# pytorch/torchdistx

Hardware: AMD Instinct MI355X
Metric: deferred_init_materialize_params_per_s (higher is better)
Workload: dtype bf16; 1 GPU; model=llama3-70b, n_params=70553706496, mode=replicate, init=fast, threads=1, replay=pertensor, device=cuda, native_init_kernels=True, parallelism=replicate1

## Files before the change

### torchdistx_amd/csrc/core/deferred_init.cc

```cpp

#include "deferred_init.h"

#include <algorithm>
#include <atomic>
#include <cmath>
#include <condition_variable>
#include <cstring>
#include <functional>
#include <limits>
#include <memory>
#include <mutex>
#include <optional>
#include <unordered_set>
#include <vector>

#include <ATen/CPUGeneratorImpl.h>
#include <ATen/Context.h>
#include <ATen/ThreadLocalState.h>
#include <c10/core/GradMode.h>
#include <ATen/core/dispatch/Dispatcher.h>
#include <ATen/core/VariableHooksInterface.h>
#include <c10/core/DefaultDtype.h>
#include <c10/core/impl/LocalDispatchKeySet.h>
#include <torch/library.h>

#include "box_geometry.h"
#include "fake.h"
#include "native_redirect.h"
#include "stack_utils.h"

namespace tdx {
namespace {

constexpr c10::DispatchKey kDeferredKey = c10::DispatchKey::DeferredInit;
constexpr c10::DispatchKey kFakeKey = c10::DispatchKey::Fake;

struct OpNode;

struct OpOutputDescriptor {
  std::shared_ptr<OpNode> node;
  size_t index = 0;
};

struct AliasGroup {
  std::vector<std::shared_ptr<OpNode>> writers;
};

struct TensorRecord {
  OpOutputDescriptor desc;
  std::shared_ptr<AliasGroup> group;
};

struct RecordedOp {
  std::string name;
  std::function<void(torch::jit::Stack&)> run;
  std::vector<c10::IValue> args;
  at::ThreadLocalState tls;
  std::optional<std::pair<uint64_t, uint64_t>> philox;
  std::optional<c10::OperatorHandle> handle;
};

constexpr uint64_t kPhiloxStridePerOp = 4;

struct RngSession {
  bool has_segment = false;
  uint64_t segment_hash = 0;
  uint64_t nonce = 0;
  uint64_t next_slot = 1;
  std::vector<uint64_t> raw_hashes;
  at::Tensor replay_cursor;
  std::mutex cursor_mutex;
};

thread_local std::shared_ptr<RngSession> current_rng_session;

std::mutex segment_registry_mutex;
std::unordered_map<uint64_t, uint64_t> live_segment_uses;

uint64_t mixSalt(uint64_t h, uint64_t salt) {
  for (int b = 0; b < 8; ++b) {
    h = (h ^ ((salt >> (8 * b)) & 0xff)) * 1099511628211ull;
  }
  return h;
}

bool isRngOpName(const std::string& name) {
  return name == "aten::uniform_" || name == "aten::normal_" ||
         name == "aten::bernoulli_";
}

uint64_t hashStateBytes(const uint8_t* bytes, int64_t n) {
  uint64_t h = 0x9E3779B97F4A7C15ull ^ static_cast<uint64_t>(n);
  int64_t i = 0;
  for (; i + 8 <= n; i += 8) {
    uint64_t w;
    std::memcpy(&w, bytes + i, 8);
    h ^= w;
    h *= 0xBF58476D1CE4E5B9ull;
    h ^= h >> 29;
  }
  uint64_t tail = 0;
  for (int j = 0; i < n; ++i, ++j) {
    tail |= static_cast<uint64_t>(bytes[i]) << (8 * j);
  }
  h ^= tail;
  h *= 0x94D049BB133111EBull;
  h ^= h >> 32;
  return h;
}

void beginRngSession() {
  current_rng_session = std::make_shared<RngSession>();
}

void endRngSession() {
  std::lock_guard<std::mutex> reg_lock(segment_registry_mutex);
  if (current_rng_session != nullptr) {
    for (uint64_t h : current_rng_session->raw_hashes) {
      auto it = live_segment_uses.find(h);
      if (it != live_segment_uses.end() && --(it->second) == 0) {
        live_segment_uses.erase(it);
      }
    }
  }
  current_rng_session = nullptr;
  auto gen = at::globalContext().defaultGenerator(c10::DeviceType::CPU);
  std::lock_guard<std::mutex> lock(gen.mutex());
  gen.get<at::CPUGeneratorImpl>()->random64();
}

std::optional<std::pair<uint64_t, uint64_t>> pinPhiloxForOp(
    const std::string& name, at::Tensor* segment_start) {
  if (!isRngOpName(name) || current_rng_session == nullptr) {
    return std::nullopt;
  }
  RngSession& session = *current_rng_session;
  std::lock_guard<std::mutex> reg_lock(segment_registry_mutex);
  auto gen = at::globalContext().defaultGenerator(c10::DeviceType::CPU);
  at::Tensor state;
  {
    std::lock_guard<std::mutex> lock(gen.mutex());
    state = gen.get_state();
  }
  const uint64_t h =
      hashStateBytes(state.const_data_ptr<uint8_t>(), state.numel());
  if (!session.has_segment || h != session.segment_hash) {
    session.has_segment = true;
    session.segment_hash = h;
    session.next_slot = 1;
    const uint64_t salt = live_segment_uses[h]++;
    session.raw_hashes.push_back(h);
    session.nonce = salt == 0 ? h : mixSalt(h, salt);
    if (salt != 0) {
      auto salted = at::make_generator<at::CPUGeneratorImpl>(session.nonce);
      state = salted.get_state();
    }
    *segment_start = std::move(state);
  }
  return std::make_pair(session.nonce,
                        session.next_slot++ * kPhiloxStridePerOp);
}

struct InputSlot {
  std::optional<OpOutputDescriptor> desc;
  std::optional<uint32_t> external_version;
  std::vector<std::shared_ptr<OpNode>> history;
  bool inference = false;
};

struct AliasGroup;

struct OpNode {
  uint64_t op_nr = 0;
  std::optional<RecordedOp> op;
  std::vector<InputSlot> input_slots;
  std::vector<c10::Storage> output_storages;
  struct OutputMeta {
    c10::ScalarType dtype = c10::ScalarType::Undefined;
    c10::Device device{c10::DeviceType::CPU};
    bool contiguous = false;
    int64_t storage_offset = 0;
    int64_t numel = 0;
  };
  std::vector<OutputMeta> output_metas;
  std::weak_ptr<OpNode> set_data_prior;
  std::vector<std::weak_ptr<OpNode>> dependents;
  std::vector<std::weak_ptr<AliasGroup>> write_groups;
  std::vector<at::Tensor> outputs;
  bool materialized = false;
  bool running = false;
};

std::atomic<uint64_t> next_op_nr{1};

std::recursive_mutex tape_mutex;
std::condition_variable_any tape_cv;

std::shared_ptr<TensorRecord> getRecord(FakeTensorImpl* fake) {
  return std::static_pointer_cast<TensorRecord>(fake->getData(kDeferredKey));
}

void setRecord(FakeTensorImpl* fake, std::shared_ptr<TensorRecord> rec) {
  fake->setData(kDeferredKey, std::move(rec));
}

uint32_t tensorVersion(const at::Tensor& t) {
  return t.unsafeGetTensorImpl()->version_counter().current_version();
}

bool storagesAlias(const c10::Storage& a, const c10::Storage& b) {
  return a && b && a.is_alias_of(b);
}


thread_local size_t deferred_level = 0;

bool shouldRecordHere() {
  return deferred_level > 0 &&
         !c10::impl::tls_is_dispatch_key_excluded(kDeferredKey);
}

void recordOp(std::string name,
              std::function<void(torch::jit::Stack&)> run,
              std::vector<c10::IValue> args,
              at::ThreadLocalState tls,
              torch::jit::Stack& stack,
              size_t rets_begin,
              std::optional<std::pair<uint64_t, uint64_t>> philox =
                  std::nullopt,
              std::optional<c10::OperatorHandle> handle = std::nullopt,
              std::weak_ptr<OpNode> set_data_prior = {}) {
  std::lock_guard<std::recursive_mutex> lock{tape_mutex};
  auto node = std::make_shared<OpNode>();
  node->set_data_prior = std::move(set_data_prior);
  node->op_nr = next_op_nr.fetch_add(1, std::memory_order_relaxed);

  std::vector<std::shared_ptr<TensorRecord>> input_records;
  std::vector<c10::Storage> input_storages;
  std::vector<size_t> fake_slot_idx;
  {
    torch::jit::Stack args_stack{args.begin(), args.end()};
    mapTensors(args_stack, 0, args_stack.size(),
               [&](const at::Tensor& t) -> at::Tensor {
                 if (auto* fake = asFake(t)) {
                   auto rec = getRecord(fake);
                   TORCH_CHECK(
                       rec != nullptr,
                       "A fake tensor constructed outside of a deferred-init "
                       "context (or stripped of its record) was used in `",
                       name, "` and cannot be recorded.");
                   fake_slot_idx.push_back(node->input_slots.size());
                   node->input_slots.push_back(InputSlot{rec->desc, {}, {}});
                   rec->desc.node->dependents.emplace_back(node);
                   input_records.push_back(std::move(rec));
                   input_storages.push_back(fake->meta_tensor().storage());
                   return at::Tensor{};
                 }
                 if (t.defined() && t.is_inference()) {
                   InputSlot slot;
                   slot.inference = true;
                   node->input_slots.push_back(std::move(slot));
                 } else if (t.defined()) {
                   node->input_slots.push_back(
                       InputSlot{{}, tensorVersion(t), {}});
                 } else {
                   node->input_slots.push_back(InputSlot{});
                 }
                 return t;
               });
    args.assign(args_stack.begin(), args_stack.end());
  }

  node->op = RecordedOp{std::move(name), std::move(run), std::move(args),
                        std::move(tls), philox, std::move(handle)};

  visitTensors(stack, rets_begin, stack.size(), [&](const at::Tensor& t) {
    size_t out_idx = node->output_storages.size();
    auto* fake = asFake(t);
    if (fake == nullptr) {
      node->output_storages.emplace_back();
      node->output_metas.emplace_back();
      return;
    }
    const c10::Storage& out_storage = fake->meta_tensor().storage();
    node->output_storages.push_back(out_storage);
    node->output_metas.push_back(OpNode::OutputMeta{
        fake->meta_tensor().scalar_type(), fake->fake_device(),
        fake->meta_tensor().is_contiguous(),
        fake->meta_tensor().storage_offset(), fake->meta_tensor().numel()});

    auto rec = getRecord(fake);
    if (rec == nullptr) {
      rec = std::make_shared<TensorRecord>();
      setRecord(fake, rec);
    }
    rec->desc = OpOutputDescriptor{node, out_idx};

    if (rec->group == nullptr) {
      for (size_t i = 0; i < input_records.size(); ++i) {
        if (storagesAlias(out_storage, input_storages[i]) &&
            input_records[i]->group != nullptr) {
          rec->group = input_records[i]->group;
          break;
        }
      }
      if (rec->group == nullptr) {
        rec->group = std::make_shared<AliasGroup>();
      }
    }
    if (rec->group->writers.empty() ||
        rec->group->writers.back() != node) {
      rec->group->writers.push_back(node);
      node->write_groups.emplace_back(rec->group);
    }
  });

  for (size_t i = 0; i < input_records.size(); ++i) {
    bool writes_it = false;
    for (const c10::Storage& out : node->output_storages) {
      if (storagesAlias(out, input_storages[i])) {
        writes_it = true;
        break;
      }
// ... 337 lines not shown
  recordOp(
      "tdx::set_data",
      [](torch::jit::Stack& s) {
        at::Tensor nd = s.back().toTensor();
        s.pop_back();
        at::Tensor slf = s.back().toTensor();
        s.pop_back();
        slf.set_data(nd);
        s.emplace_back(slf);
      },
      std::move(args), at::ThreadLocalState{}, rets, 0, std::nullopt,
      std::nullopt, std::move(prior));
}


bool outputsAlias(const OpNode& node, const c10::Storage& storage) {
  for (const c10::Storage& s : node.output_storages) {
    if (storagesAlias(s, storage)) {
      return true;
    }
  }
  return false;
}

struct CallStack {
  std::vector<std::shared_ptr<OpNode>> nodes;
  std::unordered_set<OpNode*> members;

  void addWithDeps(const std::shared_ptr<OpNode>& n) {
    if (!members.insert(n.get()).second) {
      return;
    }
    nodes.push_back(n);
    for (const InputSlot& slot : n->input_slots) {
      if (slot.desc.has_value()) {
        addWithDeps(slot.desc->node);
      }
      for (const auto& h : slot.history) {
        addWithDeps(h);
      }
    }
    for (const auto& wg : n->write_groups) {
      if (auto group = wg.lock()) {
        for (const auto& w : group->writers) {
          if (w->op_nr < n->op_nr) {
            addWithDeps(w);
          }
        }
      }
    }
  }
};

std::vector<std::shared_ptr<OpNode>> buildCallStack(const TensorRecord& rec) {
  CallStack cs;
  uint64_t horizon = 0;
  if (rec.group != nullptr) {
    for (const auto& w : rec.group->writers) {
      horizon = std::max(horizon, w->op_nr);
      cs.addWithDeps(w);
    }
  } else {
    cs.addWithDeps(rec.desc.node);
    horizon = rec.desc.node->op_nr;
  }

  bool changed = true;
  while (changed) {
    changed = false;
    std::vector<std::shared_ptr<OpNode>> snapshot = cs.nodes;
    for (const auto& n : snapshot) {
      for (const auto& wd : n->dependents) {
        auto d = wd.lock();
        if (!d || cs.members.count(d.get()) != 0 || d->materialized ||
            d->op_nr > horizon) {
          continue;
        }
        bool include = false;
        for (const InputSlot& slot : d->input_slots) {
          if (!slot.desc.has_value() ||
              cs.members.count(slot.desc->node.get()) == 0) {
            continue;
          }
          const c10::Storage& s =
              slot.desc->node->output_storages[slot.desc->index];
          if (!s) {
            continue;
          }
          for (const auto& w : cs.nodes) {
            if (w->op_nr > d->op_nr && w.get() != slot.desc->node.get() &&
                outputsAlias(*w, s)) {
              include = true;
              break;
            }
          }
          if (include) {
            break;
          }
        }
        if (include) {
          cs.addWithDeps(d);
          changed = true;
        }
      }
    }
  }

  std::sort(cs.nodes.begin(), cs.nodes.end(),
            [](const auto& a, const auto& b) { return a->op_nr < b->op_nr; });
  return cs.nodes;
}

torch::jit::Stack materializeArguments(OpNode& node) {
  torch::jit::Stack stack{node.op->args.begin(), node.op->args.end()};
  size_t visit = 0;
  mapTensors(stack, 0, stack.size(), [&](const at::Tensor& t) -> at::Tensor {
    const InputSlot& slot = node.input_slots.at(visit++);
    if (slot.desc.has_value()) {
      const OpOutputDescriptor& dep = *slot.desc;
      TORCH_INTERNAL_ASSERT(dep.node->materialized,
                            "deferred-init replay ordering bug: dependency "
                            "not yet materialized");
      return dep.node->outputs.at(dep.index);
    }
    TORCH_CHECK(!slot.inference,
                "An inference tensor was used while recording `",
                node.op->name,
                "`; in-place updates to inference tensors cannot be "
                "tracked, so the tape cannot be replayed faithfully.");
    if (t.defined() && slot.external_version.has_value()) {
      TORCH_CHECK(tensorVersion(t) == *slot.external_version,
                  "The external tensor used by the recorded op `",
                  node.op->name,
                  "` was modified in place after recording; the tape can no "
                  "longer be replayed faithfully.");
    }
    return t;
  });
  return stack;
}

void replayNode(std::unique_lock<std::recursive_mutex>& lock,
                const std::shared_ptr<OpNode>& node) {
  while (node->running) {
    tape_cv.wait(lock);
  }
  if (node->materialized) {
    return;
  }
  TORCH_CHECK(node->op.has_value(),
              "This deferred-init tape segment has already been freed and "
              "cannot be replayed again.");
  torch::jit::Stack stack = materializeArguments(*node);
  node->running = true;
  lock.unlock();
  try {
    at::ThreadLocalStateGuard tls_guard{node->op->tls};
    c10::impl::ExcludeDispatchKeyGuard no_deferred{kDeferredKey};
    c10::impl::ExcludeDispatchKeyGuard no_fake{kFakeKey};
    node->op->run(stack);
  } catch (...) {
    lock.lock();
    node->running = false;
    tape_cv.notify_all();
    throw;
  }
  lock.lock();
  node->running = false;
  node->outputs.clear();
  visitTensors(stack, 0, stack.size(),
               [&](const at::Tensor& t) { node->outputs.push_back(t); });
  node->materialized = true;
  node->op.reset();
  node->input_slots.clear();
  node->input_slots.shrink_to_fit();
  tape_cv.notify_all();
}

}

void enterDeferredInit() {
  if (deferred_level++ == 0) {
    beginRngSession();
    c10::impl::tls_set_dispatch_key_included(kDeferredKey, true);
    installProxyHooks();
  }
}

void leaveDeferredInit() {
  TORCH_CHECK(deferred_level > 0, "Not in a deferred-init context.");
  if (--deferred_level == 0) {
    c10::impl::tls_set_dispatch_key_included(kDeferredKey, false);
    removeProxyHooks();
    endRngSession();
  }
}

bool isDeferredInitActive() noexcept {
  return deferred_level > 0;
}

NoDeferredInit::NoDeferredInit()
    : prev_{c10::impl::tls_is_dispatch_key_excluded(kDeferredKey)} {
  c10::impl::tls_set_dispatch_key_excluded(kDeferredKey, true);
}

NoDeferredInit::~NoDeferredInit() {
  c10::impl::tls_set_dispatch_key_excluded(kDeferredKey, prev_);
}

// ... 1229 lines not shown
  for (int64_t d = 0; d < dim; ++d) {
    n_blocks *= meta.size(d);
  }
  const ShardWindow w{n_blocks, (end_row - start_row) * inner,
                      dim_len * inner, start_row * inner};

  std::vector<int64_t> shard_sizes(meta.sizes().begin(), meta.sizes().end());
  if (!shard_sizes.empty()) {
    shard_sizes[dim] = end_row - start_row;
  }
  return replayChainOnShard(fake, shard_sizes, w);
}

at::Tensor materializeTensorBlock(const at::Tensor& tensor,
                                  at::IntArrayRef starts,
                                  at::IntArrayRef ends) {
  auto* fake = asFake(tensor);
  TORCH_CHECK_VALUE(fake != nullptr && getRecord(fake) != nullptr,
                    "`tensor` is not a deferred tensor.");
  const at::Tensor& meta = fake->meta_tensor();
  TORCH_CHECK(meta.is_contiguous(),
              "slice materialization requires a contiguous tensor");
  const int64_t rank = meta.dim();
  TORCH_CHECK(static_cast<int64_t>(starts.size()) == rank &&
                  static_cast<int64_t>(ends.size()) == rank,
              "block materialization takes one start and one end per dim: "
              "got ", starts.size(), " and ", ends.size(), " for a ", rank,
              "-d tensor");
  std::vector<int64_t> shard_sizes(rank);
  for (int64_t d = 0; d < rank; ++d) {
    TORCH_CHECK(0 <= starts[d] && starts[d] <= ends[d] &&
                    ends[d] <= meta.size(d),
                "invalid slice range [", starts[d], ", ", ends[d],
                ") for size ", meta.size(d), " along dim ", d);
    shard_sizes[d] = ends[d] - starts[d];
  }
  BoxGeometry box;
  const BoxStatus status = normalizeBox(meta.sizes().data(), starts.data(),
                                        ends.data(), static_cast<int>(rank),
                                        &box);
  TORCH_CHECK(status == BoxStatus::kOk,
              "slice materialization: the block needs more than ",
              kMaxBoxLevels, " nested strided levels; materialize the "
              "tensor fully instead.");
  ShardWindow w{1, box.run_len, box.run_len, box.g_off};
  if (box.levels == 1) {
    w = ShardWindow{box.extent[0], box.run_len, box.g_stride[0], box.g_off};
  } else if (box.levels >= 2) {
    w.box = box;
  }
  return replayChainOnShard(fake, shard_sizes, w);
}

at::Tensor materializeTensor(const at::Tensor& tensor) {
  auto* fake = asFake(tensor);
  if (fake == nullptr) {
    return tensor;
  }
  auto rec = getRecord(fake);
  TORCH_CHECK_VALUE(rec != nullptr,
                    "`tensor` is fake but carries no deferred-init record, "
                    "so it cannot be materialized.");

  std::unique_lock<std::recursive_mutex> lock{tape_mutex};
  OpOutputDescriptor desc = rec->desc;
  for (const auto& n : buildCallStack(*rec)) {
    replayNode(lock, n);
  }

  at::Tensor out = desc.node->outputs.at(desc.index);
  if (out.is_leaf() && out.requires_grad() != tensor.requires_grad()) {
    out.set_requires_grad(tensor.requires_grad());
  }
  return out;
}

}
```

### torchdistx_amd/csrc/core/deferred_init.h

```cpp

#pragma once

#include <ATen/ATen.h>

namespace tdx {

void enterDeferredInit();
void leaveDeferredInit();
bool isDeferredInitActive() noexcept;

class NoDeferredInit {
 public:
  NoDeferredInit();
  ~NoDeferredInit();
  NoDeferredInit(const NoDeferredInit&) = delete;
  NoDeferredInit& operator=(const NoDeferredInit&) = delete;

 private:
  bool prev_;
};

bool canMaterialize(const at::Tensor& tensor) noexcept;

at::Tensor materializeTensor(const at::Tensor& tensor);

struct RecordInfo {
  uint64_t op_nr = 0;
  size_t output_index = 0;
  bool materialized = false;
  std::string op_name;
  size_t pending_ops = 0;
};

std::optional<RecordInfo> recordInfo(const at::Tensor& tensor);

struct InitPlan {
  enum class Kind { kFactory, kUniform, kNormal, kBernoulli, kFill, kZero };
  Kind kind = Kind::kFactory;
  double p0 = 0.0;
  double p1 = 0.0;
  uint64_t seed = 0;
  uint64_t offset = 0;
  std::vector<int64_t> sizes;
  c10::ScalarType dtype = c10::ScalarType::Float;
  std::optional<c10::ScalarType> src_dtype;
  c10::Device device{c10::DeviceType::CPU};
  bool requires_grad = false;
};

std::optional<InitPlan> tensorInitPlan(const at::Tensor& tensor);

struct TailOp {
  enum Code : int32_t {
    kErfinv = 0,
    kMul = 1,
    kAdd = 2,
    kSub = 3,
    kClamp = 4,
    kClampMin = 5,
    kClampMax = 6,
    kNeg = 7,
    kAbs = 8,
  };
  int32_t op = kErfinv;
  double s0 = 0.0;
  double s1 = 0.0;
};

constexpr size_t kMaxTailOps = 8;

const char* tailOpName(int32_t op);

struct ChainPlan : InitPlan {
  std::vector<TailOp> tail;
};

std::optional<ChainPlan> tensorChainPlan(const at::Tensor& tensor);
// ... 28 lines not shown
```

### torchdistx_amd/csrc/core/fake.cc

```cpp

#include "fake.h"

#include <mutex>

#include <ATen/core/dispatch/Dispatcher.h>
#include <c10/core/DeviceGuard.h>
#include <c10/core/impl/DeviceGuardImplInterface.h>
#include <c10/core/impl/FakeGuardImpl.h>
#include <c10/core/impl/LocalDispatchKeySet.h>
#include <torch/library.h>

#include "stack_utils.h"

namespace tdx {
namespace {

constexpr c10::DispatchKey kFakeKey = c10::DispatchKey::Fake;

c10::Device canonicalFakeDevice(c10::Device d) {
  if (d.is_cuda() && !d.has_index()) {
    const auto* guard =
        c10::impl::device_guard_impl_registry[static_cast<size_t>(
                                                  c10::DeviceType::CUDA)]
            .load();
// ... 80 lines not shown

FakeTensorImpl* asFake(const at::Tensor& tensor) noexcept {
  if (!tensor.defined() ||
      !tensor.unsafeGetTensorImpl()->key_set().has(kFakeKey)) {
    return nullptr;
  }
  return dynamic_cast<FakeTensorImpl*>(tensor.unsafeGetTensorImpl());
}

bool isFake(const at::Tensor& tensor) noexcept {
  return asFake(tensor) != nullptr;
}

at::Tensor makeFake(at::Tensor meta, c10::Device fake_device) {
  return at::detail::make_tensor<FakeTensorImpl>(std::move(meta),
                                                 fake_device);
}

at::Tensor metaLike(const at::Tensor& fake) {
  auto* impl = asFake(fake);
  TORCH_CHECK_VALUE(impl != nullptr,
                    "`fake` was expected to be a fake tensor.");
  return at::Tensor{impl->meta_tensor().unsafeGetTensorImpl()
                        ->shallow_copy_and_detach(
                            0,
                            true)};
}


namespace {

bool isDeviceType(const c10::TypePtr& type) {
  if (type->kind() == c10::TypeKind::DeviceObjType) {
    return true;
  }
  if (type->kind() == c10::TypeKind::OptionalType) {
    return type->castRaw<c10::OptionalType>()->getElementType()->kind() ==
           c10::TypeKind::DeviceObjType;
  }
  return false;
}

struct FakeCall {
  const c10::OperatorHandle& op;
  torch::jit::Stack* stack;
  size_t args_begin;
  size_t num_args;

  bool has_tensor_arg = false;
  bool has_fake_arg = false;
  std::optional<c10::Device> tensor_device;
  std::optional<size_t> device_arg_slot;
  std::optional<c10::Device> explicit_device;
  std::unordered_map<c10::TensorImpl*, at::Tensor> meta_to_fake;
};

bool opConsumesDeviceArg(const c10::OperatorHandle& op) {
  if (op.hasKernelForDispatchKey(c10::DispatchKey::BackendSelect)) {
    return true;
  }
  const auto& args = op.schema().arguments();
  for (size_t i = 0; i + 3 < args.size(); ++i) {
    if (args[i].name() == "dtype" && args[i + 1].name() == "layout" &&
        args[i + 2].name() == "device" &&
        args[i + 3].name() == "pin_memory") {
      return true;
    }
  }
  return false;
}

void assessOp(FakeCall& call) {
  const auto& schema = call.op.schema();

  visitTensors(
      *call.stack, call.args_begin, call.args_begin + call.num_args,
      [&](const at::Tensor& t) {
        if (!t.defined()) {
          return;
        }
        call.has_tensor_arg = true;
        if (isFake(t)) {
          call.has_fake_arg = true;
        }
        if (t.dim() == 0 && t.device().is_cpu()) {
          return;
        }
        c10::Device d = t.device();
        if (!call.tensor_device.has_value()) {
          call.tensor_device = d;
        } else {
          TORCH_CHECK(*call.tensor_device == d, "`", schema.operator_name(),
                      "` was called on fake tensors with arguments spread "
                      "over two devices (", *call.tensor_device, " and ", d,
                      "); fake dispatch needs one common device (0-dim CPU "
                      "scalars excepted).");
        }
      });

  if (!opConsumesDeviceArg(call.op)) {
    return;
  }
  const auto& args = schema.arguments();
  for (size_t i = 0; i < args.size(); ++i) {
    if (args[i].name() == "device" && isDeviceType(args[i].type())) {
      call.device_arg_slot = i;
      const c10::IValue& v = (*call.stack)[call.args_begin + i];
// ... 5 lines not shown
  }
}

c10::Device outputDevice(const FakeCall& call) {
  if (call.explicit_device.has_value()) {
    return *call.explicit_device;
  }
  if (call.tensor_device.has_value()) {
    return *call.tensor_device;
  }
  return c10::Device{c10::DeviceType::CPU};
}

void fakeHandler(const c10::OperatorHandle& op,
                 c10::DispatchKeySet ks,
                 torch::jit::Stack* stack) {
  c10::impl::ExcludeDispatchKeyGuard no_reentry{kFakeKey};

  const auto& schema = op.schema();
  size_t num_args = schema.arguments().size();
  size_t num_rets = schema.returns().size();

  FakeCall call{op, stack, stack->size() - num_args, num_args};
  assessOp(call);

  bool should_fake = call.has_fake_arg || call.device_arg_slot.has_value() ||
                     !call.has_tensor_arg;
  if (!should_fake) {
    op.redispatchBoxed(
        ks & c10::DispatchKeySet{c10::DispatchKeySet::FULL_AFTER, kFakeKey},
        stack);
    return;
  }

  c10::Device out_device = outputDevice(call);

  TORCH_CHECK(op.hasComputedKernelForDispatchKey(c10::DispatchKey::Meta),
              "`", schema.operator_name(),
              "` has no meta-backend kernel, so it cannot run on fake "
              "tensors.");
  if (!out_device.is_meta()) {
    c10::DispatchKey backend_key = c10::computeDispatchKey(
        std::nullopt, std::nullopt, out_device);
    TORCH_CHECK(op.hasComputedKernelForDispatchKey(backend_key),
                "`", schema.operator_name(), "` has no kernel for '",
                out_device, "', so its fake result could never be "
                "materialized on that device.");
  }

  mapTensors(*stack, call.args_begin, call.args_begin + num_args,
             [&](const at::Tensor& t) -> at::Tensor {
               if (auto* fake = asFake(t)) {
                 const at::Tensor& shadow = fake->meta_tensor();
                 call.meta_to_fake.emplace(shadow.unsafeGetTensorImpl(), t);
                 return shadow;
               }
               return t;
             });
  if (call.device_arg_slot.has_value()) {
    (*stack)[call.args_begin + *call.device_arg_slot] =
        c10::IValue{c10::Device{c10::DeviceType::Meta}};
  }

  op.redispatchBoxed(c10::DispatchKeySet{c10::DispatchKey::Meta}, stack);

  mapTensors(*stack, stack->size() - num_rets, stack->size(),
             [&](const at::Tensor& t) -> at::Tensor {
               if (!t.defined() || !t.is_meta()) {
                 return t;
               }
               auto it = call.meta_to_fake.find(t.unsafeGetTensorImpl());
               if (it != call.meta_to_fake.end()) {
                 asFake(it->second)->refreshFromMeta();
                 return it->second;
               }
               return makeFake(t, out_device);
             });
}

TORCH_LIBRARY_IMPL(_, Fake, m) {
  m.fallback(torch::CppFunction::makeFromBoxedFunction<&fakeHandler>());
}


thread_local size_t fake_mode_level = 0;

std::mutex guard_mutex;
size_t fake_cuda_entries = 0;
bool installed_fake_cuda_guard = false;

std::atomic<const c10::impl::DeviceGuardImplInterface*>& cudaGuardSlot() {
  return c10::impl::device_guard_impl_registry[static_cast<size_t>(
      c10::DeviceType::CUDA)];
}

void pushFakeCudaGuard() {
  std::lock_guard<std::mutex> lock{guard_mutex};
  if (fake_cuda_entries++ == 0 && cudaGuardSlot().load() == nullptr) {
    static c10::impl::FakeGuardImpl<c10::DeviceType::CUDA> noop_guard;
    cudaGuardSlot().store(&noop_guard);
    installed_fake_cuda_guard = true;
  }
}

void popFakeCudaGuard() {
  std::lock_guard<std::mutex> lock{guard_mutex};
  if (fake_cuda_entries > 0 && --fake_cuda_entries == 0 &&
      installed_fake_cuda_guard) {
    cudaGuardSlot().store(nullptr);
    installed_fake_cuda_guard = false;
  }
}

thread_local bool fake_cuda_active = false;

}

void enterFakeMode(bool fake_cuda) {
  if (fake_mode_level++ == 0) {
    c10::impl::tls_set_dispatch_key_included(kFakeKey, true);
    if (fake_cuda) {
      pushFakeCudaGuard();
      fake_cuda_active = true;
    }
  }
}

// ... 17 lines not shown
```

### torchdistx_amd/csrc/core/fake.h

```cpp

#pragma once

#include <memory>
#include <unordered_map>

#include <ATen/ATen.h>
#include <c10/core/TensorImpl.h>

namespace tdx {

class FakeTensorImpl : public c10::TensorImpl {
 public:
  FakeTensorImpl(at::Tensor meta, c10::Device fake_device);

  const at::Tensor& meta_tensor() const noexcept {
    return meta_;
  }

  c10::Device fake_device() const noexcept {
    return fake_device_;
  }

  void refreshFromMeta();

  void setData(c10::DispatchKey key, std::shared_ptr<void> data) {
    dispatch_data_[key] = std::move(data);
  }
  std::shared_ptr<void> getData(c10::DispatchKey key) const {
    auto it = dispatch_data_.find(key);
    return it == dispatch_data_.end() ? nullptr : it->second;
  }
  bool hasData(c10::DispatchKey key) const {
    return dispatch_data_.count(key) != 0;
  }

  c10::intrusive_ptr<TensorImpl> shallow_copy_and_detach(
      const c10::VariableVersion& version_counter,
      bool allow_tensor_metadata_change) const override;
  c10::intrusive_ptr<TensorImpl> shallow_copy_and_detach(
      c10::VariableVersion&& version_counter,
      bool allow_tensor_metadata_change) const override;
  void shallow_copy_from(const c10::intrusive_ptr<TensorImpl>& impl) override;

 private:
  template <typename VariableVersion>
  c10::intrusive_ptr<TensorImpl> shallowCopyAndDetachImpl(
      VariableVersion&& version_counter,
      bool allow_tensor_metadata_change) const;

  at::Tensor meta_;
  c10::Device fake_device_;
  std::unordered_map<c10::DispatchKey, std::shared_ptr<void>> dispatch_data_;
};

FakeTensorImpl* asFake(const at::Tensor& tensor) noexcept;

bool isFake(const at::Tensor& tensor) noexcept;

at::Tensor makeFake(at::Tensor meta, c10::Device fake_device);

at::Tensor metaLike(const at::Tensor& fake);

void enterFakeMode(bool fake_cuda);
void leaveFakeMode();
bool isFakeModeActive() noexcept;

}
```

### torchdistx_amd/csrc/core/module.cc

```cpp

#include <torch/extension.h>

#include <torch/csrc/utils/device_lazy_init.h>

#include "deferred_init.h"
#include "fake.h"
#include "native_redirect.h"

namespace {

thread_local size_t fake_cuda_lazy_init_suppressions = 0;

void enterFakeModeBinding(bool fake_cuda) {
  if (fake_cuda) {
    torch::utils::set_requires_device_init(at::kCUDA, false);
    ++fake_cuda_lazy_init_suppressions;
  }
  tdx::enterFakeMode(fake_cuda);
}

pybind11::object srcDtypeObject(const tdx::InitPlan& plan) {
  if (!plan.src_dtype.has_value()) {
    return pybind11::none();
  }
// ... 25 lines not shown

  m.def("enter_fake_mode", &enterFakeModeBinding, pybind11::arg("fake_cuda"),
        "Enter fake-tensor mode on this thread (nestable). With fake_cuda, "
        "fake \"cuda\" tensors can be built without a GPU runtime.");
  m.def("leave_fake_mode", &leaveFakeModeBinding,
        "Leave the innermost fake mode.");

  m.def("is_fake", [](const at::Tensor& t) { return tdx::isFake(t); },
        "Whether the tensor is a storage-less fake tensor.");

  m.def("meta_like", [](const at::Tensor& t) { return tdx::metaLike(t); },
        "Detached meta tensor with the fake tensor's metadata; raises "
        "ValueError for non-fake inputs.");

  m.def("enter_deferred_init", &tdx::enterDeferredInit,
        "Enter deferred-init recording on this thread (nestable).");
  m.def("leave_deferred_init", &tdx::leaveDeferredInit,
        "Leave the innermost deferred-init context.");

  m.def("can_materialize",
        [](const at::Tensor& t) { return tdx::canMaterialize(t); },
        "Whether the tensor is fake AND carries a replayable tape record.");

  m.def("set_native_init", &tdx::setNativeInitEnabled,
        pybind11::arg("enabled"));
  m.def("native_init_enabled", &tdx::nativeInitEnabled);
  m.def("set_native_init_cpu", &tdx::setNativeInitCpuEnabled,
        pybind11::arg("enabled"));
  m.def("native_init_cpu_enabled", &tdx::nativeInitCpuEnabled);

  m.def("record_info", [](const at::Tensor& t) -> pybind11::object {
    auto info = tdx::recordInfo(t);
    if (!info.has_value()) {
      return pybind11::none();
    }
    pybind11::dict d;
    d["op_nr"] = info->op_nr;
    d["output_index"] = info->output_index;
    d["materialized"] = info->materialized;
    d["op_name"] = info->op_name;
    d["pending_ops"] = info->pending_ops;
    return d;
  });

  m.def("materialize_tensor", [](const at::Tensor& t) {
    at::Tensor out;
    {
      pybind11::gil_scoped_release release;
      out = tdx::materializeTensor(t);
    }
    return out;
  }, "Replays the tensor's tape segment (GIL released); identity for real "
     "tensors, stable object across repeated calls and aliases.");

  m.def("tensor_init_plan", [](const at::Tensor& t) -> pybind11::object {
    auto plan = tdx::tensorInitPlan(t);
    if (!plan.has_value()) {
      return pybind11::none();
    }
    static const char* kKinds[] = {"factory", "uniform", "normal",
                                   "bernoulli", "fill", "zero"};
    pybind11::dict d;
    d["kind"] = kKinds[static_cast<int>(plan->kind)];
    d["p0"] = plan->p0;
    d["p1"] = plan->p1;
    d["seed"] = static_cast<int64_t>(plan->seed);
    d["offset"] = static_cast<int64_t>(plan->offset);
    d["sizes"] = plan->sizes;
    d["dtype"] = pybind11::cast(plan->dtype);
    d["src_dtype"] = srcDtypeObject(*plan);
    d["device"] = pybind11::cast(plan->device);
    d["requires_grad"] = plan->requires_grad;
    return d;
  }, "Reduced replay plan of a simple init chain (the final whole-tensor "
     "value step), or None when the tape is not that simple. \"dtype\" is "
     "the final dtype; \"src_dtype\" is the dtype an RNG step was recorded "
     "at when a conversion follows it, else None. Feeds the "
     "batched replay planner (materialize_module_batched).");

  m.def("set_fused_init_chains", &tdx::setFusedInitChains,
        pybind11::arg("enabled"));
  m.def("fused_init_chains_enabled", &tdx::fusedInitChainsEnabled);
  m.def("reset_fused_init_chains", &tdx::resetFusedInitChains,
        "Back to the start-up state: TDX_FUSED_INIT_CHAINS if set, else on "
        "by default (not explicitly).");
  m.def("fused_init_chains_explicit", &tdx::fusedInitChainsExplicit,
        "True once fusion was switched on explicitly; only then does what "
        "is not bitwise equal to ATen's kernels fuse: erfinv_ on float32 "
        "(and float16 mul_ on tensors of 2^31 elements or more).");

  m.def("tensor_chain_plan", [](const at::Tensor& t) -> pybind11::object {
    auto plan = tdx::tensorChainPlan(t);
    if (!plan.has_value()) {
      return pybind11::none();
    }
    static const char* kKinds[] = {"factory", "uniform", "normal",
                                   "bernoulli", "fill", "zero"};
    pybind11::dict d;
    d["kind"] = kKinds[static_cast<int>(plan->kind)];
    d["p0"] = plan->p0;
    d["p1"] = plan->p1;
    d["seed"] = static_cast<int64_t>(plan->seed);
    d["offset"] = static_cast<int64_t>(plan->offset);
    d["sizes"] = plan->sizes;
    d["dtype"] = pybind11::cast(plan->dtype);
    d["src_dtype"] = srcDtypeObject(*plan);
// ... 92 lines not shown
```

### torchdistx_amd/csrc/core/native_redirect.cc

```cpp
#include "native_redirect.h"

#include <atomic>
#include <cstdlib>
#include <cstring>

namespace tdx {
namespace {

std::atomic<bool> native_init_enabled{true};
std::atomic<bool> native_init_cpu_enabled{false};

int fusedInitChainsDefault() {
  const char* v = std::getenv("TDX_FUSED_INIT_CHAINS");
  if (v == nullptr) {
    return 1;
  }
  return std::strcmp(v, "0") == 0 ? 0 : 2;
}

std::atomic<int> fused_init_chains_mode{fusedInitChainsDefault()};

struct Redirect {
  const char* aten_name;
  const char* aten_overload;
  const char* tdx_name;
  bool needs_float_dtype;
};

constexpr Redirect kRedirects[] = {
    {"aten::uniform_", "", "uniform_", true},
    {"aten::normal_", "", "normal_", true},
    {"aten::bernoulli_", "float", "bernoulli_", true},
    {"aten::fill_", "Scalar", "fill_", true},
    {"aten::zero_", "", "zero_", false},
    {"aten::copy_", "", "copy_", true},
};

bool requireNative() {
  static const bool required = std::getenv("TDX_REQUIRE_NATIVE_INIT") != nullptr;
  return required;
}

}

void setNativeInitEnabled(bool enabled) noexcept {
  native_init_enabled.store(enabled, std::memory_order_relaxed);
}

bool nativeInitEnabled() noexcept {
  return native_init_enabled.load(std::memory_order_relaxed);
}

void setNativeInitCpuEnabled(bool enabled) noexcept {
  native_init_cpu_enabled.store(enabled, std::memory_order_relaxed);
}

bool nativeInitCpuEnabled() noexcept {
  return native_init_cpu_enabled.load(std::memory_order_relaxed);
}

void setFusedInitChains(bool enabled) noexcept {
  fused_init_chains_mode.store(enabled ? 2 : 0, std::memory_order_relaxed);
}

void resetFusedInitChains() noexcept {
  fused_init_chains_mode.store(fusedInitChainsDefault(),
                               std::memory_order_relaxed);
}

bool fusedInitChainsEnabled() noexcept {
  return fused_init_chains_mode.load(std::memory_order_relaxed) != 0;
}

bool fusedInitChainsExplicit() noexcept {
  return fused_init_chains_mode.load(std::memory_order_relaxed) == 2;
}

bool tryNativeInitRedirect(
    const c10::OperatorHandle& op,
    torch::jit::Stack& stack,
    const std::optional<std::pair<uint64_t, uint64_t>>& philox) {
  if (!nativeInitEnabled()) {
    return false;
  }
  const auto& name = op.schema().operator_name();
  const Redirect* redirect = nullptr;
  for (const Redirect& r : kRedirects) {
    if (name.name == r.aten_name && name.overload_name == r.aten_overload) {
      redirect = &r;
      break;
    }
  }
  if (redirect == nullptr) {
    return false;
  }

  if (stack.empty() || !stack.front().isTensor()) {
    return false;
  }
  const at::Tensor& self = stack.front().toTensor();
  if (!self.defined() || !self.is_contiguous()) {
    return false;
  }
  if (!self.is_cuda() && !(self.is_cpu() && nativeInitCpuEnabled())) {
    return false;
  }
  if (redirect->needs_float_dtype) {
    auto st = self.scalar_type();
    if (st != at::kFloat && st != at::kBFloat16 && st != at::kHalf) {
      return false;
    }
  }
  if (std::strcmp(redirect->tdx_name, "copy_") == 0) {
    if (stack.size() < 2 || !stack[1].isTensor()) {
      return false;
    }
    const at::Tensor& src = stack[1].toTensor();
    auto sst = src.scalar_type();
    if (!src.defined() || src.device() != self.device() ||
        !src.is_contiguous() || !src.sizes().equals(self.sizes()) ||
        (sst != at::kFloat && sst != at::kBFloat16 && sst != at::kHalf)) {
      return false;
    }
  }

  auto target = c10::Dispatcher::singleton().findOp(
      {std::string("tdx::") + redirect->tdx_name, ""});
  if (!target.has_value()) {
    TORCH_CHECK(!requireNative(),
                "TDX_REQUIRE_NATIVE_INIT is set but the torchdistx_amd._K "
                "kernel extension is not loaded; refusing to fall back to "
                "stock ATen kernels for `",
                name, "`.");
    return false;
  }
  const bool is_rng = std::strcmp(redirect->tdx_name, "uniform_") == 0 ||
                      std::strcmp(redirect->tdx_name, "normal_") == 0 ||
                      std::strcmp(redirect->tdx_name, "bernoulli_") == 0;
  if (is_rng) {
    for (const c10::IValue& v : stack) {
      if (v.isGenerator()) {
        return false;
      }
    }
    if (philox.has_value()) {
      stack.emplace_back(static_cast<int64_t>(philox->first));
      stack.emplace_back(static_cast<int64_t>(philox->second));
    } else {
      stack.emplace_back();
      stack.emplace_back();
    }
  }
  target->callBoxed(&stack);
  return true;
}

}
```

### torchdistx_amd/csrc/core/stack_utils.h

```cpp

#pragma once

#include <functional>

#include <ATen/core/ivalue.h>
#include <ATen/core/stack.h>

namespace tdx {

using TensorVisitor = std::function<void(const at::Tensor&)>;

void visitTensors(const torch::jit::Stack& stack,
                  size_t begin,
                  size_t end,
                  const TensorVisitor& visitor);

using TensorMapFn = std::function<at::Tensor(const at::Tensor&)>;

void mapTensors(torch::jit::Stack& stack,
                size_t begin,
                size_t end,
                const TensorMapFn& fn);

std::vector<c10::IValue> copyStackRegion(const torch::jit::Stack& stack,
                                         size_t begin,
                                         size_t end);

}
```

### torchdistx_amd/deferred_init.py

```python

from typing import Callable, Dict, Optional, TypeVar, Union


from torch import Tensor
from torch.nn import Module, Parameter
from torch.utils.weak import WeakTensorKeyDictionary

from torchdistx_amd import fake
from torchdistx_amd import _C

T = TypeVar("T", bound=Module)

_wrapper_memo: "WeakTensorKeyDictionary" = WeakTensorKeyDictionary()

_worker_streams: list = []


def deferred_init(module_fn: Callable[..., T], *args, **kwargs) -> T:
    _C.enter_deferred_init()
    try:
        return module_fn(*args, **kwargs)
    finally:
        _C.leave_deferred_init()


def is_deferred(obj: Union[Tensor, Module]) -> bool:
    if isinstance(obj, Tensor):
        return _C.can_materialize(obj)

    if isinstance(obj, Module):
        return any(
            _C.can_materialize(t)
            for t in list(obj.parameters()) + list(obj.buffers())
        )

    raise ValueError("`obj` must be of type `Tensor` or `Module`.")


def materialize_tensor(tensor: Tensor) -> Tensor:
    materialized = _C.materialize_tensor(tensor)
    if materialized is tensor:
        return tensor
    return _restore_class(tensor, materialized)


def _restore_class(original: Tensor, materialized: Tensor) -> Tensor:
    cls = type(original)
    if cls is type(materialized):
        return materialized
    wrapper = _wrapper_memo.get(materialized)
    if wrapper is None or type(wrapper) is not cls:
        if cls is Parameter:
            wrapper = Parameter(
                materialized, requires_grad=original.requires_grad
            )
        else:
            wrapper = materialized.as_subclass(cls)
            if (
                wrapper.is_leaf
                and wrapper.requires_grad != original.requires_grad
            ):
                wrapper.requires_grad_(original.requires_grad)
        _wrapper_memo[materialized] = wrapper
    return wrapper


def materialize_module(
    module: Module,
    buffers_only: bool = False,
    check_fn: Optional[Callable[[Module], bool]] = None,
) -> None:

    def swap(tensors: Dict[str, Optional[Tensor]]) -> None:
        for key, tensor in tensors.items():
            if tensor is None:
                continue
            try:
                tensors[key] = materialize_tensor(tensor)
            except ValueError:
                raise ValueError(
                    f"'{key}' has already been materialized."
                ) from None

    for child in module.children():
        materialize_module(child, buffers_only, check_fn)

    if check_fn is None or check_fn(module):
        if not buffers_only:
            swap(module._parameters)
        swap(module._buffers)


_DIST_CODE = {"uniform": 0, "normal": 1, "bernoulli": 2, "fill": 3,
              "zero": 4, "factory": -1}

_TAIL_CODE = {"erfinv": 0, "mul": 1, "add": 2, "sub": 3, "clamp": 4,
              "clamp_min": 5, "clamp_max": 6, "neg": 7, "abs": 8}


def materialize_module_batched(
    module: Module,
    buffers_only: bool = False,
    check_fn: Optional[Callable[[Module], bool]] = None,
    device=None,
) -> None:
    import torch

    from torchdistx_amd import _kernels

    entries = []
    for submodule in module.modules():
        if check_fn is not None and not check_fn(submodule):
            continue
        if not buffers_only:
            for key, p in submodule._parameters.items():
                if p is not None and _C.can_materialize(p):
                    entries.append((submodule, key, p, True))
        for key, b in submodule._buffers.items():
            if b is not None and _C.can_materialize(b):
                entries.append((submodule, key, b, False))

    for entry in _batched_fill(entries, device=device):
        submodule, key, tensor, is_param = entry
        mat = materialize_tensor(tensor)
        if device is not None and mat.device != torch.device(device):
            moved = mat.detach().to(device)
            moved.requires_grad_(mat.requires_grad)
            mat = _restore_class(tensor, moved)
        if is_param:
            submodule._parameters[key] = mat
        else:
            submodule._buffers[key] = mat


def _same_device(a, b) -> bool:
    return a.type == b.type and (
        a.index is None or b.index is None or a.index == b.index
    )


def _batched_fill(entries, device=None) -> list:
    import torch

# ... 199 lines not shown
```

Before: 1674 billion params/s.

## Cut host overhead in deferred-init record and replay paths

Bundles several host-side reductions. It caches the RNG state hash by comparing raw generator fields instead of serializing and hashing the state for every RNG op, and adds a fast call-stack path for small closed writer chains. It batches module materialization into a single C++ call with one GIL release, one tape-lock acquisition and one TLS install scope, and caches native redirect lookup and target resolution. It also swaps small unordered_maps for linear vectors, std::function for function_ref, and drops an args stack copy. The risks are subtle behaviour changes: TLS is no longer restored between nodes, the fast chain path may skip dependencies, and the batched path's fallback on ValueError may double-materialize.

```diff
diff --git a/torchdistx_amd/csrc/core/deferred_init.cc b/torchdistx_amd/csrc/core/deferred_init.cc
--- a/torchdistx_amd/csrc/core/deferred_init.cc
+++ b/torchdistx_amd/csrc/core/deferred_init.cc
@@ -11,6 +11,7 @@
 #include <memory>
 #include <mutex>
 #include <optional>
+#include <unordered_map>
 #include <unordered_set>
 #include <vector>
 
@@ -62,12 +63,41 @@
 
 constexpr uint64_t kPhiloxStridePerOp = 4;
 
+struct GeneratorFields {
+  at::mt19937_data_pod engine;
+  std::optional<float> next_float;
+  std::optional<double> next_double;
+
+  static GeneratorFields read(at::CPUGeneratorImpl& gen) {
+    return GeneratorFields{gen.engine().data(),
+                           gen.next_float_normal_sample(),
+                           gen.next_double_normal_sample()};
+  }
+
+  bool sameAs(const GeneratorFields& o) const {
+    auto same_bits = [](const auto& a, const auto& b) {
+      return a.has_value() == b.has_value() &&
+             (!a.has_value() || std::memcmp(&*a, &*b, sizeof(*a)) == 0);
+    };
+    return engine.seed_ == o.engine.seed_ && engine.left_ == o.engine.left_ &&
+           engine.seeded_ == o.engine.seeded_ &&
+           engine.next_ == o.engine.next_ &&
+           std::memcmp(engine.state_.data(), o.engine.state_.data(),
+                       sizeof(engine.state_)) == 0 &&
+           same_bits(next_float, o.next_float) &&
+           same_bits(next_double, o.next_double);
+  }
+};
+
 struct RngSession {
   bool has_segment = false;
   uint64_t segment_hash = 0;
   uint64_t nonce = 0;
   uint64_t next_slot = 1;
   std::vector<uint64_t> raw_hashes;
+  bool has_last = false;
+  GeneratorFields last_fields;
+  uint64_t last_hash = 0;
   at::Tensor replay_cursor;
   std::mutex cursor_mutex;
 };
@@ -138,13 +168,23 @@
   std::lock_guard<std::mutex> reg_lock(segment_registry_mutex);
   auto gen = at::globalContext().defaultGenerator(c10::DeviceType::CPU);
   at::Tensor state;
+  uint64_t h = 0;
   {
     std::lock_guard<std::mutex> lock(gen.mutex());
-    state = gen.get_state();
-  }
-  const uint64_t h =
-      hashStateBytes(state.const_data_ptr<uint8_t>(), state.numel());
+    GeneratorFields fields =
+        GeneratorFields::read(*gen.get<at::CPUGeneratorImpl>());
+    if (session.has_last && fields.sameAs(session.last_fields)) {
+      h = session.last_hash;
+    } else {
+      state = gen.get_state();
+      h = hashStateBytes(state.const_data_ptr<uint8_t>(), state.numel());
+      session.has_last = true;
+      session.last_fields = fields;
+      session.last_hash = h;
+    }
+  }
   if (!session.has_segment || h != session.segment_hash) {
+    TORCH_INTERNAL_ASSERT(state.defined());
     session.has_segment = true;
     session.segment_hash = h;
     session.next_slot = 1;
@@ -239,8 +279,8 @@
   std::vector<c10::Storage> input_storages;
   std::vector<size_t> fake_slot_idx;
   {
-    torch::jit::Stack args_stack{args.begin(), args.end()};
-    mapTensors(args_stack, 0, args_stack.size(),
+    node->input_slots.reserve(args.size());
+    mapTensors(args, 0, args.size(),
                [&](const at::Tensor& t) -> at::Tensor {
                  if (auto* fake = asFake(t)) {
                    auto rec = getRecord(fake);
@@ -268,7 +308,6 @@
                  }
                  return t;
                });
-    args.assign(args_stack.begin(), args_stack.end());
   }
 
   node->op = RecordedOp{std::move(name), std::move(run), std::move(args),
@@ -712,7 +751,58 @@
   }
 };
 
+bool closedChainCallStack(const std::shared_ptr<AliasGroup>& group,
+                          std::vector<std::shared_ptr<OpNode>>* out) {
+  constexpr size_t kMaxClosedChain = 8;
+  const auto& writers = group->writers;
+  if (writers.empty() || writers.size() > kMaxClosedChain) {
+    return false;
+  }
+  auto is_writer = [&writers](const OpNode* n) {
+    for (const auto& w : writers) {
+      if (w.get() == n) {
+        return true;
+      }
+    }
+    return false;
+  };
+  const uint64_t horizon = writers.back()->op_nr;
+  uint64_t prev_nr = 0;
+  for (const auto& w : writers) {
+    if (w->op_nr <= prev_nr) {
+      return false;
+    }
+    prev_nr = w->op_nr;
+    if (w->write_groups.size() != 1 ||
+        w->write_groups[0].owner_before(group) ||
+        group.owner_before(w->write_groups[0])) {
+      return false;
+    }
+    for (const InputSlot& slot : w->input_slots) {
+      if (!slot.history.empty() ||
+          (slot.desc.has_value() && !is_writer(slot.desc->node.get()))) {
+        return false;
+      }
+    }
+    for (const auto& wd : w->dependents) {
+      auto d = wd.lock();
+      if (d && !d->materialized && d->op_nr <= horizon &&
+          !is_writer(d.get())) {
+        return false;
+      }
+    }
+  }
+  out->assign(writers.begin(), writers.end());
+  return true;
+}
+
 std::vector<std::shared_ptr<OpNode>> buildCallStack(const TensorRecord& rec) {
+  if (rec.group != nullptr) {
+    std::vector<std::shared_ptr<OpNode>> chain;
+    if (closedChainCallStack(rec.group, &chain)) {
+      return chain;
+    }
+  }
   CallStack cs;
   uint64_t horizon = 0;
   if (rec.group != nullptr) {
@@ -800,7 +890,30 @@
   return stack;
 }
 
+class ReplayTlsScope {
+ public:
+  ReplayTlsScope() = default;
+  ReplayTlsScope(const ReplayTlsScope&) = delete;
+  ReplayTlsScope& operator=(const ReplayTlsScope&) = delete;
+  ~ReplayTlsScope() {
+    if (caller_.has_value()) {
+      at::ThreadLocalState::setThreadLocalState(*caller_);
+    }
+  }
+
+  void install(const at::ThreadLocalState& recorded) {
+    if (!caller_.has_value()) {
+      caller_.emplace();
+    }
+    at::ThreadLocalState::setThreadLocalState(recorded);
+  }
+
+ private:
+  std::optional<at::ThreadLocalState> caller_;
+};
+
 void replayNode(std::unique_lock<std::recursive_mutex>& lock,
+                ReplayTlsScope& tls_scope,
                 const std::shared_ptr<OpNode>& node) {
   while (node->running) {
     tape_cv.wait(lock);
@@ -815,7 +928,7 @@
   node->running = true;
   lock.unlock();
   try {
-    at::ThreadLocalStateGuard tls_guard{node->op->tls};
+    tls_scope.install(node->op->tls);
     c10::impl::ExcludeDispatchKeyGuard no_deferred{kDeferredKey};
     c10::impl::ExcludeDispatchKeyGuard no_fake{kFakeKey};
     node->op->run(stack);
@@ -2151,7 +2264,11 @@
   return replayChainOnShard(fake, shard_sizes, w);
 }
 
-at::Tensor materializeTensor(const at::Tensor& tensor) {
+namespace {
+
+at::Tensor materializeLocked(std::unique_lock<std::recursive_mutex>& lock,
+                             ReplayTlsScope& tls_scope,
+                             const at::Tensor& tensor) {
   auto* fake = asFake(tensor);
   if (fake == nullptr) {
     return tensor;
@@ -2161,10 +2278,9 @@
                     "`tensor` is fake but carries no deferred-init record, "
                     "so it cannot be materialized.");
 
-  std::unique_lock<std::recursive_mutex> lock{tape_mutex};
   OpOutputDescriptor desc = rec->desc;
   for (const auto& n : buildCallStack(*rec)) {
-    replayNode(lock, n);
+    replayNode(lock, tls_scope, n);
   }
 
   at::Tensor out = desc.node->outputs.at(desc.index);
@@ -2175,3 +2291,26 @@
 }
 
 }
+
+at::Tensor materializeTensor(const at::Tensor& tensor) {
+  if (asFake(tensor) == nullptr) {
+    return tensor;
+  }
+  ReplayTlsScope tls_scope;
+  std::unique_lock<std::recursive_mutex> lock{tape_mutex};
+  return materializeLocked(lock, tls_scope, tensor);
+}
+
+std::vector<at::Tensor> materializeTensors(
+    const std::vector<at::Tensor>& tensors) {
+  std::vector<at::Tensor> out;
+  out.reserve(tensors.size());
+  ReplayTlsScope tls_scope;
+  std::unique_lock<std::recursive_mutex> lock{tape_mutex};
+  for (const at::Tensor& t : tensors) {
+    out.push_back(materializeLocked(lock, tls_scope, t));
+  }
+  return out;
+}
+
+}
diff --git a/torchdistx_amd/csrc/core/deferred_init.h b/torchdistx_amd/csrc/core/deferred_init.h
--- a/torchdistx_amd/csrc/core/deferred_init.h
+++ b/torchdistx_amd/csrc/core/deferred_init.h
@@ -23,6 +23,9 @@
 bool canMaterialize(const at::Tensor& tensor) noexcept;
 
 at::Tensor materializeTensor(const at::Tensor& tensor);
+
+std::vector<at::Tensor> materializeTensors(
+    const std::vector<at::Tensor>& tensors);
 
 struct RecordInfo {
   uint64_t op_nr = 0;
diff --git a/torchdistx_amd/csrc/core/fake.cc b/torchdistx_amd/csrc/core/fake.cc
--- a/torchdistx_amd/csrc/core/fake.cc
+++ b/torchdistx_amd/csrc/core/fake.cc
@@ -156,7 +156,16 @@
   std::optional<c10::Device> tensor_device;
   std::optional<size_t> device_arg_slot;
   std::optional<c10::Device> explicit_device;
-  std::unordered_map<c10::TensorImpl*, at::Tensor> meta_to_fake;
+  std::vector<std::pair<c10::TensorImpl*, at::Tensor>> meta_to_fake;
+
+  const at::Tensor* fakeOf(c10::TensorImpl* meta_impl) const {
+    for (const auto& entry : meta_to_fake) {
+      if (entry.first == meta_impl) {
+        return &entry.second;
+      }
+    }
+    return nullptr;
+  }
 };
 
 bool opConsumesDeviceArg(const c10::OperatorHandle& op) {
@@ -268,7 +277,10 @@
              [&](const at::Tensor& t) -> at::Tensor {
                if (auto* fake = asFake(t)) {
                  const at::Tensor& shadow = fake->meta_tensor();
-                 call.meta_to_fake.emplace(shadow.unsafeGetTensorImpl(), t);
+                 if (call.fakeOf(shadow.unsafeGetTensorImpl()) == nullptr) {
+                   call.meta_to_fake.emplace_back(
+                       shadow.unsafeGetTensorImpl(), t);
+                 }
                  return shadow;
                }
                return t;
@@ -285,10 +297,10 @@
                if (!t.defined() || !t.is_meta()) {
                  return t;
                }
-               auto it = call.meta_to_fake.find(t.unsafeGetTensorImpl());
-               if (it != call.meta_to_fake.end()) {
-                 asFake(it->second)->refreshFromMeta();
-                 return it->second;
+               if (const at::Tensor* fake =
+                       call.fakeOf(t.unsafeGetTensorImpl())) {
+                 asFake(*fake)->refreshFromMeta();
+                 return *fake;
                }
                return makeFake(t, out_device);
              });
diff --git a/torchdistx_amd/csrc/core/fake.h b/torchdistx_amd/csrc/core/fake.h
--- a/torchdistx_amd/csrc/core/fake.h
+++ b/torchdistx_amd/csrc/core/fake.h
@@ -2,7 +2,8 @@
 #pragma once
 
 #include <memory>
-#include <unordered_map>
+#include <utility>
+#include <vector>
 
 #include <ATen/ATen.h>
 #include <c10/core/TensorImpl.h>
@@ -24,14 +25,29 @@
   void refreshFromMeta();
 
   void setData(c10::DispatchKey key, std::shared_ptr<void> data) {
-    dispatch_data_[key] = std::move(data);
+    for (auto& entry : dispatch_data_) {
+      if (entry.first == key) {
+        entry.second = std::move(data);
+        return;
+      }
+    }
+    dispatch_data_.emplace_back(key, std::move(data));
   }
   std::shared_ptr<void> getData(c10::DispatchKey key) const {
-    auto it = dispatch_data_.find(key);
-    return it == dispatch_data_.end() ? nullptr : it->second;
+    for (const auto& entry : dispatch_data_) {
+      if (entry.first == key) {
+        return entry.second;
+      }
+    }
+    return nullptr;
   }
   bool hasData(c10::DispatchKey key) const {
-    return dispatch_data_.count(key) != 0;
+    for (const auto& entry : dispatch_data_) {
+      if (entry.first == key) {
+        return true;
+      }
+    }
+    return false;
   }
 
   c10::intrusive_ptr<TensorImpl> shallow_copy_and_detach(
@@ -50,7 +66,8 @@
 
   at::Tensor meta_;
   c10::Device fake_device_;
-  std::unordered_map<c10::DispatchKey, std::shared_ptr<void>> dispatch_data_;
+  std::vector<std::pair<c10::DispatchKey, std::shared_ptr<void>>>
+      dispatch_data_;
 };
 
 FakeTensorImpl* asFake(const at::Tensor& tensor) noexcept;
diff --git a/torchdistx_amd/csrc/core/module.cc b/torchdistx_amd/csrc/core/module.cc
--- a/torchdistx_amd/csrc/core/module.cc
+++ b/torchdistx_amd/csrc/core/module.cc
@@ -101,6 +101,17 @@
     return out;
   }, "Replays the tensor's tape segment (GIL released); identity for real "
      "tensors, stable object across repeated calls and aliases.");
+
+  m.def("materialize_tensors", [](const std::vector<at::Tensor>& ts) {
+    std::vector<at::Tensor> out;
+    {
+      pybind11::gil_scoped_release release;
+      out = tdx::materializeTensors(ts);
+    }
+    return out;
+  }, pybind11::arg("tensors"),
+     "materialize_tensor over a list, in order, with one GIL release and "
+     "one tape-lock acquisition for the whole list.");
 
   m.def("tensor_init_plan", [](const at::Tensor& t) -> pybind11::object {
     auto plan = tdx::tensorInitPlan(t);
diff --git a/torchdistx_amd/csrc/core/native_redirect.cc b/torchdistx_amd/csrc/core/native_redirect.cc
--- a/torchdistx_amd/csrc/core/native_redirect.cc
+++ b/torchdistx_amd/csrc/core/native_redirect.cc
@@ -3,6 +3,9 @@
 #include <atomic>
 #include <cstdlib>
 #include <cstring>
+#include <mutex>
+#include <optional>
+#include <unordered_map>
 
 namespace tdx {
 namespace {
@@ -76,6 +79,56 @@
   return fused_init_chains_mode.load(std::memory_order_relaxed) == 2;
 }
 
+namespace {
+
+constexpr size_t kNumRedirects = sizeof(kRedirects) / sizeof(kRedirects[0]);
+
+bool isRngRedirect(const Redirect& r) {
+  return std::strcmp(r.tdx_name, "uniform_") == 0 ||
+         std::strcmp(r.tdx_name, "normal_") == 0 ||
+         std::strcmp(r.tdx_name, "bernoulli_") == 0;
+}
+
+int redirectIndex(const c10::OperatorHandle& op) {
+  thread_local std::unordered_map<c10::OperatorHandle, int> table;
+  auto it = table.find(op);
+  if (it != table.end()) {
+    return it->second;
+  }
+  const auto& name = op.schema().operator_name();
+  int index = -1;
+  for (size_t i = 0; i < kNumRedirects; ++i) {
+    if (name.name == kRedirects[i].aten_name &&
+        name.overload_name == kRedirects[i].aten_overload) {
+      index = static_cast<int>(i);
+      break;
+    }
+  }
+  table.emplace(op, index);
+  return index;
+}
+
+const c10::OperatorHandle* redirectTarget(int index) {
+  static std::mutex mutex;
+  static std::optional<c10::OperatorHandle> targets[kNumRedirects];
+  static std::atomic<bool> resolved[kNumRedirects];
+  if (!resolved[index].load(std::memory_order_acquire)) {
+    std::lock_guard<std::mutex> lock{mutex};
+    if (!resolved[index].load(std::memory_order_relaxed)) {
+      auto target = c10::Dispatcher::singleton().findOp(
+          {std::string("tdx::") + kRedirects[index].tdx_name, ""});
+      if (!target.has_value()) {
+        return nullptr;
+      }
+      targets[index] = *target;
+      resolved[index].store(true, std::memory_order_release);
+    }
+  }
+  return &*targets[index];
+}
+
+}
+
 bool tryNativeInitRedirect(
     const c10::OperatorHandle& op,
     torch::jit::Stack& stack,
@@ -83,17 +136,11 @@
   if (!nativeInitEnabled()) {
     return false;
   }
-  const auto& name = op.schema().operator_name();
-  const Redirect* redirect = nullptr;
-  for (const Redirect& r : kRedirects) {
-    if (name.name == r.aten_name && name.overload_name == r.aten_overload) {
-      redirect = &r;
-      break;
-    }
-  }
-  if (redirect == nullptr) {
-    return false;
-  }
+  const int index = redirectIndex(op);
+  if (index < 0) {
+    return false;
+  }
+  const Redirect* redirect = &kRedirects[index];
 
   if (stack.empty() || !stack.front().isTensor()) {
     return false;
@@ -124,19 +171,16 @@
     }
   }
 
-  auto target = c10::Dispatcher::singleton().findOp(
-      {std::string("tdx::") + redirect->tdx_name, ""});
-  if (!target.has_value()) {
+  const c10::OperatorHandle* target = redirectTarget(index);
+  if (target == nullptr) {
     TORCH_CHECK(!requireNative(),
                 "TDX_REQUIRE_NATIVE_INIT is set but the torchdistx_amd._K "
                 "kernel extension is not loaded; refusing to fall back to "
                 "stock ATen kernels for `",
-                name, "`.");
-    return false;
-  }
-  const bool is_rng = std::strcmp(redirect->tdx_name, "uniform_") == 0 ||
-                      std::strcmp(redirect->tdx_name, "normal_") == 0 ||
-                      std::strcmp(redirect->tdx_name, "bernoulli_") == 0;
+                op.schema().operator_name(), "`.");
+    return false;
+  }
+  const bool is_rng = isRngRedirect(*redirect);
   if (is_rng) {
     for (const c10::IValue& v : stack) {
       if (v.isGenerator()) {
diff --git a/torchdistx_amd/csrc/core/stack_utils.h b/torchdistx_amd/csrc/core/stack_utils.h
--- a/torchdistx_amd/csrc/core/stack_utils.h
+++ b/torchdistx_amd/csrc/core/stack_utils.h
@@ -1,21 +1,20 @@
 
 #pragma once
 
-#include <functional>
-
 #include <ATen/core/ivalue.h>
 #include <ATen/core/stack.h>
+#include <c10/util/FunctionRef.h>
 
 namespace tdx {
 
-using TensorVisitor = std::function<void(const at::Tensor&)>;
+using TensorVisitor = c10::function_ref<void(const at::Tensor&)>;
 
 void visitTensors(const torch::jit::Stack& stack,
                   size_t begin,
                   size_t end,
                   const TensorVisitor& visitor);
 
-using TensorMapFn = std::function<at::Tensor(const at::Tensor&)>;
+using TensorMapFn = c10::function_ref<at::Tensor(const at::Tensor&)>;
 
 void mapTensors(torch::jit::Stack& stack,
                 size_t begin,
diff --git a/torchdistx_amd/deferred_init.py b/torchdistx_amd/deferred_init.py
--- a/torchdistx_amd/deferred_init.py
+++ b/torchdistx_amd/deferred_init.py
@@ -1,5 +1,5 @@
 
-from typing import Callable, Dict, Optional, TypeVar, Union
+from typing import Callable, Dict, List, Optional, Tuple, TypeVar, Union
 
 
 from torch import Tensor
@@ -65,30 +65,47 @@
     return wrapper
 
 
+_Slots = List[Tuple[Dict[str, Optional[Tensor]], str, Tensor]]
+
+
+def _collect_slots(
+    module: Module,
+    buffers_only: bool,
+    check_fn: Optional[Callable[[Module], bool]],
+    slots: _Slots,
+) -> None:
+    for child in module.children():
+        _collect_slots(child, buffers_only, check_fn, slots)
+    if check_fn is None or check_fn(module):
+        groups = (module._buffers,) if buffers_only else (
+            module._parameters, module._buffers)
+        for tensors in groups:
+            for key, tensor in tensors.items():
+                if tensor is not None:
+                    slots.append((tensors, key, tensor))
+
+
 def materialize_module(
     module: Module,
     buffers_only: bool = False,
     check_fn: Optional[Callable[[Module], bool]] = None,
 ) -> None:
-
-    def swap(tensors: Dict[str, Optional[Tensor]]) -> None:
-        for key, tensor in tensors.items():
-            if tensor is None:
-                continue
+    slots: _Slots = []
+    _collect_slots(module, buffers_only, check_fn, slots)
+    try:
+        materialized = _C.materialize_tensors([s[2] for s in slots])
+    except ValueError:
+        for tensors, key, tensor in slots:
             try:
                 tensors[key] = materialize_tensor(tensor)
             except ValueError:
                 raise ValueError(
                     f"'{key}' has already been materialized."
                 ) from None
-
-    for child in module.children():
-        materialize_module(child, buffers_only, check_fn)
-
-    if check_fn is None or check_fn(module):
-        if not buffers_only:
-            swap(module._parameters)
-        swap(module._buffers)
+        raise
+    for (tensors, key, tensor), mat in zip(slots, materialized):
+        if mat is not tensor:
+            tensors[key] = _restore_class(tensor, mat)
 
 
 _DIST_CODE = {"uniform": 0, "normal": 1, "bernoulli": 2, "fill": 3,
```

After: 1584 billion params/s. 5.3% lower.
